# RajeshRk18/exacto

Measured on AMD Instinct MI355X. Metric: ciphertext muls/sec (bfv_mul_and_relin), higher is better.
Workload: dtype u64; 1 GPU; bfv_mul_and_relin, BASELINE configs[2]; ring_degree=4096, ct_limbs=3, limb_bits=60, plain_modulus=65537, gadget_base=65536, gadget_digits=12, batch_per_gpu=1024, global_batch=1024, parallelism=batch-shard x1

## Files before the change

exacto_amd/csrc/ks32.hip:

```cpp
#include "exacto_internal.hpp"
#include "ks32_dev.hpp"

#include <algorithm>

namespace exacto {


template <int LOGN, typename DT, int FORM>
__global__ void __launch_bounds__((1 << LOGN) / 16)
ks32_digit_ntt_kernel(const DT* __restrict__ D16, uint32_t* __restrict__ DS, int G, int S,
                      const Prime32* __restrict__ primes) {
    constexpr int N = 1 << LOGN, T = N / 16;
    __shared__ uint32_t lds[N];
    const int tid = threadIdx.x;
    const uint32_t b = blockIdx.x;
    const int s = (int)(b % (uint32_t)S);
    const long ig = b / (uint32_t)S;
    const Prime32& P = primes[s];
    const DT* src = D16 + ig * N;
    uint32_t x[16];
    constexpr bool SIN = FORM == F32_LAZY && sizeof(DT) == 2;
#pragma unroll
    for (int k = 0; k < 16; ++k) {
        const int d = src[tid + k * T];
        x[k] = SIN ? (uint32_t)d : d < 0 ? P.p + (uint32_t)d : (uint32_t)d;
    }
    fwd32_store<LOGN, FORM, SIN, FORM != F32_LAZY>(x, lds, tid, P, DS + (long)b * N);
}

template <int LOGN, int FORM>
__global__ void __launch_bounds__((1 << LOGN) / 16)
ks32_key_kernel(const u64* __restrict__ K, uint32_t* __restrict__ RS, int L, int S,
                const Prime32* __restrict__ primes, const PrimeConst* __restrict__ qprimes) {
    constexpr int N = 1 << LOGN, T = N / 16;
    __shared__ uint32_t lds[N];
    const int tid = threadIdx.x;
    const uint32_t b = blockIdx.x;
    const int s = (int)(b % (uint32_t)S);
    const uint32_t row = b / (uint32_t)S;
    const int l = (int)(row % (uint32_t)L);
    const Prime32& P = primes[s];
    const u64 q = qprimes[l].q, half = q >> 1;
    const u64* src = K + (long)row * N;
    uint32_t x[16];
#pragma unroll
    for (int k = 0; k < 16; ++k) {
        const u64 r = src[tid + k * T];
        if (r > half) {
            const uint32_t m = (uint32_t)((q - r) % P.p);
            x[k] = m == 0 ? 0 : P.p - m;
        } else {
            x[k] = (uint32_t)(r % P.p);
        }
    }
    fwd32_store<LOGN, FORM>(x, lds, tid, P, RS + (long)b * N);
}

__global__ void __launch_bounds__(256)
ks32_key_norm_kernel(const u64* __restrict__ K, u64* __restrict__ out, int L, int n,
                     const PrimeConst* __restrict__ qprimes) {
    __shared__ u64 part[256];
    const uint32_t row = blockIdx.x;
    const u64 q = qprimes[row % (uint32_t)L].q, half = q >> 1;
    const u64* src = K + (long)row * n;
    u64 acc = 0;
    for (int j = threadIdx.x; j < n; j += 256) {
        const u64 r = src[j];
        acc += (r > half ? q - r : r) >> 20;
    }
    part[threadIdx.x] = acc;
    __syncthreads();
    for (int w = 128; w > 0; w >>= 1) {
        if ((int)threadIdx.x < w) part[threadIdx.x] += part[threadIdx.x + w];
        __syncthreads();
    }
    if (threadIdx.x == 0) out[row] = part[0];
}

__device__ __forceinline__ uint32_t red_s64(long long x, const Prime32& P) {
    const uint32_t p = P.p;
    const uint32_t hu = (uint32_t)((unsigned long long)x >> 32) ^ 0x80000000u;
    const uint32_t a = red32(shoup32(hu, P.c32, P.c32s, p), p);
    const uint32_t b = red32(red32((uint32_t)x, 2 * p), p);
    return red32(red32(a + b, p) + P.k63, p);
}

__device__ __forceinline__ uint32_t red_s64_lz(long long x, const Prime32& P) {
    const uint32_t p = P.p;
    const uint32_t hu = (uint32_t)((unsigned long long)x >> 32) ^ 0x80000000u;
    const uint32_t a = red32(shoup32(hu, P.c32, P.c32s, p), p);
    const uint32_t lo = (uint32_t)x;
    const uint32_t b = lo - (lo >> 30) * p;
    const uint32_t s = a + b + P.k63;
    return min(s, s - 2 * p);
}

__device__ __forceinline__ long long red_s64_lazy(long long x, const Prime32& P) {
    const uint32_t hu = (uint32_t)((unsigned long long)x >> 32) ^ 0x80000000u;
    const uint32_t a = shoup32(hu, P.c32, P.c32s, P.p);
    return (long long)((unsigned long long)a + (uint32_t)x + P.k63);
}

constexpr int KS_LS = 64;
template <int CLB, int NW, int RUN, bool LZ = false>
__global__ void __launch_bounds__(NW * 64)
ks32_mac_kernel(const int* __restrict__ DS, const int* __restrict__ RS, uint32_t* __restrict__ U,
                int G, int CL, int S, int items, int n, const Prime32* __restrict__ primes) {
    extern __shared__ int kl[];
    constexpr int IG = 4 * NW;
    const int lane = threadIdx.x & (KS_LS - 1);
    const int wave = __builtin_amdgcn_readfirstlane(threadIdx.x / KS_LS);
    const int nb = n / KS_LS;
    const int jb = blockIdx.x % nb;
    const int s = (blockIdx.x / nb) % S;
    const int cl0 = (blockIdx.x / (nb * S)) * CLB;
    const int j = jb * KS_LS + lane;
    const Prime32& P = primes[s];
    for (int rr = wave; rr < G * CLB; rr += NW) {
        const int g = rr / CLB, c = rr - g * CLB;
        kl[rr * KS_LS + lane] = RS[(((long)g * CL + cl0 + c) * S + s) * n + jb * KS_LS + lane];
    }
    __syncthreads();
    const int it_end = min(items, (int)(blockIdx.y + 1) * IG);
    for (int it = blockIdx.y * IG + wave; it < it_end; it += NW) {
        const int* dp = DS + ((long)it * G * S + s) * n + j;
        long long acc[CLB];
#pragma unroll
        for (int c = 0; c < CLB; ++c) acc[c] = 0;
        for (int g0 = 0; g0 < G; g0 += RUN) {
            int d[RUN];
#pragma unroll
            for (int e = 0; e < RUN; ++e) d[e] = dp[(long)min(g0 + e, G - 1) * S * n];
#pragma unroll
            for (int e = 0; e < RUN; ++e) d[e] = g0 + e < G ? d[e] : 0;
#pragma unroll
            for (int e = 0; e < RUN; ++e) {
                const int* kg = kl + (min(g0 + e, G - 1) * CLB) * KS_LS + lane;
#pragma unroll
                for (int c = 0; c < CLB; ++c) acc[c] += (long long)d[e] * kg[c * KS_LS];
            }
            if (g0 + RUN < G) {
#pragma unroll
                for (int c = 0; c < CLB; ++c) acc[c] = red_s64_lazy(acc[c], P);
            }
        }
#pragma unroll
        for (int c = 0; c < CLB; ++c)
            U[(((long)it * CL + cl0 + c) * S + s) * n + j] = LZ ? red_s64_lz(acc[c], P) : red_s64(acc[c], P);
    }
}

template <int LOGN, int S, bool LAZY, bool FPC>
__global__ void __launch_bounds__((1 << LOGN) / 16)
ks32_crt_kernel(const uint32_t* __restrict__ U, u64* __restrict__ R, long r_stride, int L,
                const Ks32Tables* __restrict__ KT, const Prime32* __restrict__ primes,
                const PrimeConst* __restrict__ qprimes) {
    constexpr int N = 1 << LOGN, T = N / 16;
    __shared__ uint32_t lds[N];
    const int tid = threadIdx.x;
    const uint32_t b = blockIdx.x;
    u64 x[16];
    ks32_crt_values<LOGN, S, LAZY, FPC>(x, U, R, r_stride, L, b, lds, tid, KT, primes, qprimes);
    const uint32_t CL = 2 * L;
    const long item = b / CL;
    const __amdgpu_buffer_rsrc_t rd = poly_rsrc(R + item * r_stride + (long)(b - (uint32_t)item * CL) * N, N * 8);
#pragma unroll
    for (int k = 0; k < 16; ++k) buf_st64(rd, x[k], tid * 8, k * T * 8);
}

template <typename OT, typename IT>
__global__ void __launch_bounds__(256)
ks32_digit_sum_kernel(const IT* __restrict__ D, int npairs, const int* __restrict__ term_start,
                      const CombineTerm* __restrict__ terms, OT* __restrict__ out, int d, int gu, int n,
                      int nsh) {
    const uint32_t row = blockIdx.x >> nsh;
    const int j = (int)(blockIdx.x & ((1u << nsh) - 1)) * 2048 + 8 * threadIdx.x;
    const uint32_t g = row % (uint32_t)gu;
    const uint32_t ik = row / (uint32_t)gu;
    const int k = (int)(ik % (uint32_t)d);
    const long item = ik / (uint32_t)d;
    int acc[8] = {0, 0, 0, 0, 0, 0, 0, 0};
    for (int t = term_start[k]; t < term_start[k + 1]; ++t) {
        const IT* src = D + ((item * npairs + terms[t].pair) * gu + g) * (long)n + j;
        if constexpr (sizeof(IT) == 2) {
            const uint4 w = *reinterpret_cast<const uint4*>(src);
            const uint32_t v[4] = {w.x, w.y, w.z, w.w};
#pragma unroll
            for (int h = 0; h < 4; ++h) {
                acc[2 * h] += (int)(int16_t)(v[h] & 0xFFFF);
                acc[2 * h + 1] += (int)(int16_t)(v[h] >> 16);
            }
        } else {
            const uint2 w = *reinterpret_cast<const uint2*>(src);
            const uint32_t v[2] = {w.x, w.y};
#pragma unroll
            for (int h = 0; h < 8; ++h) acc[h] += (int)(int8_t)(v[h >> 2] >> (8 * (h & 3)));
        }
    }
    if constexpr (sizeof(OT) == 2) {
        uint4 o;
        uint32_t* op = &o.x;
#pragma unroll
        for (int h = 0; h < 4; ++h) op[h] = ((uint32_t)acc[2 * h] & 0xFFFF) | ((uint32_t)acc[2 * h + 1] << 16);
        *reinterpret_cast<uint4*>(out + (long)row * n + j) = o;
    } else {
        int4* o4 = reinterpret_cast<int4*>(out + (long)row * n + j);
        o4[0] = make_int4(acc[0], acc[1], acc[2], acc[3]);
        o4[1] = make_int4(acc[4], acc[5], acc[6], acc[7]);
    }
}


#define FORM_SWITCH(form, CALL)                          \
    switch (form) {                                      \
        case F32_LAZY: CALL(F32_LAZY); break;            \
        case F32_NARROW: CALL(F32_NARROW); break;        \
        default: CALL(F32_WIDE); break;                  \
    }

template <int LOGN>
static void ks32_launch_digits(const void* D, bool wide, uint32_t* DS, int items, int G, int S, const Prime32* primes,
                               int form, hipStream_t st) {
    const dim3 grid((unsigned)((long)items * G * S)), block((1 << LOGN) / 16);
#define DIG_(F_)                                                                                                \
    do {                                                                                                        \
        if (wide)                                                                                               \
            EXACTO_LAUNCH((ks32_digit_ntt_kernel<LOGN, int32_t, F_>), grid, block, 0, st, (const int32_t*)D, \
                               DS, G, S, primes);                                                               \
        else                                                                                                    \
            EXACTO_LAUNCH((ks32_digit_ntt_kernel<LOGN, int16_t, F_>), grid, block, 0, st, (const int16_t*)D, \
                               DS, G, S, primes);                                                               \
    } while (0)
    FORM_SWITCH(form, DIG_)
#undef DIG_
}

template <int LOGN>
static void ks32_launch_key(const u64* K, uint32_t* RS, long rows, int L, int S, const Prime32* primes,
                            const PrimeConst* qprimes, int form, hipStream_t st) {
#define KEY_(F_) EXACTO_LAUNCH((ks32_key_kernel<LOGN, F_>), dim3((unsigned)(rows * S)), dim3((1 << LOGN) / 16), 0, \
                                    st, K, RS, L, S, primes, qprimes)
    FORM_SWITCH(form, KEY_)
#undef KEY_
}

template <int LOGN, bool LAZY>
static void ks32_launch_crt(const uint32_t* U, u64* R, long r_stride, int items, int L, int S, const Ks32Tables* KT,
                            const Prime32* primes, const PrimeConst* qprimes, hipStream_t st, bool fpc) {
    const dim3 grid((unsigned)((long)items * 2 * L)), block((1 << LOGN) / 16);
#define CRT_(S_, F_) EXACTO_LAUNCH((ks32_crt_kernel<LOGN, S_, LAZY, F_>), grid, block, 0, st, U, R, r_stride, L, KT, \
                                   primes, qprimes)
    if (S == 2) {
        if (fpc) CRT_(2, true); else CRT_(2, false);
    } else if (S == 3) {
        if (fpc) CRT_(3, true); else CRT_(3, false);
    } else {
        if (fpc) CRT_(4, true); else CRT_(4, false);
    }
#undef CRT_
}

#define KS32_SWITCH(logn, CALL)                  \
    switch (logn) {                              \
        case 10: CALL(10); break;                \
        case 11: CALL(11); break;                \
        case 12: CALL(12); break;                \
        case 13: CALL(13); break;                \
        case 14: CALL(14); break;                \
        default: break;                          \
    }

void ks32_digits(const int16_t* D16, uint32_t* DS, int items, int G, int S, int logn, const Prime32* primes, int form,
                 hipStream_t st) {
    if (items <= 0) return;
#define CALL(L_) ks32_launch_digits<L_>(D16, false, DS, items, G, S, primes, form, st)
    KS32_SWITCH(logn, CALL)
#undef CALL
}

void ks32_digits32(const int32_t* D, uint32_t* DS, int items, int G, int S, int logn, const Prime32* primes, int form,
                   hipStream_t st) {
    if (items <= 0) return;
#define CALL(L_) ks32_launch_digits<L_>(D, true, DS, items, G, S, primes, form, st)
    KS32_SWITCH(logn, CALL)
#undef CALL
}

void ks32_key(const u64* K, uint32_t* RS, long rows, int L, int S, int logn, const Prime32* primes,
              const PrimeConst* qprimes, int form, hipStream_t st) {
    if (rows <= 0) return;
#define CALL(L_) ks32_launch_key<L_>(K, RS, rows, L, S, primes, qprimes, form, st)
    KS32_SWITCH(logn, CALL)
#undef CALL
}

void ks32_key_norms(const u64* K, u64* out, long rows, int L, int n, const PrimeConst* qprimes, hipStream_t st) {
    if (rows <= 0) return;
    EXACTO_LAUNCH(ks32_key_norm_kernel, dim3((unsigned)rows), dim3(256), 0, st, K, out, L, n, qprimes);
}

void ks32_mac(const uint32_t* DS, const uint32_t* RS, uint32_t* U, int items, int G, int L, int S, int n,
              const Prime32* primes, int mac_form, hipStream_t st) {
    if (items <= 0) return;
    const int CL = 2 * L;
    int CLB = CL;
    while (CLB > 1 && (CL % CLB != 0 || (size_t)G * CLB * KS_LS * sizeof(int) > 65536)) --CLB;
    const size_t lds = (size_t)G * CLB * KS_LS * sizeof(int);
    const int NW = lds > 32768 ? 8 : 4;
    const dim3 grid((unsigned)((n / KS_LS) * S * (CL / CLB)), (unsigned)((items + 4 * NW - 1) / (4 * NW)));
    const int* ds = reinterpret_cast<const int*>(DS);
    const int* rs = reinterpret_cast<const int*>(RS);
#define MAC_(C_, W_, R_, Z_) EXACTO_LAUNCH((ks32_mac_kernel<C_, W_, R_, Z_>), grid, dim3(W_ * 64), lds, st, ds, rs, U, G, CL, S, items, n, primes)
#define MAC(C_)                                                  \
    do {                                                         \
        if (mac_form == 2) { if (NW == 8) MAC_(C_, 8, 12, true); else MAC_(C_, 4, 12, true); } \
        else if (mac_form == 1) { if (NW == 8) MAC_(C_, 8, 12, false); else MAC_(C_, 4, 12, false); } \
        else { if (NW == 8) MAC_(C_, 8, 7, false); else MAC_(C_, 4, 7, false); }          \
    } while (0)
    switch (CLB) {
        case 8: MAC(8); break;
        case 6: MAC(6); break;
        case 4: MAC(4); break;
        case 3: MAC(3); break;
        case 2: MAC(2); break;
        default: MAC(1); break;
    }
#undef MAC
#undef MAC_
}

void ks32_digit_sum(const void* D, bool in8, int npairs, const int* term_start, const CombineTerm* terms, void* out,
                    bool wide, int items, int d, int gu, int n, hipStream_t st) {
    const long rows = (long)items * d * gu;
    if (rows <= 0) return;
    const int nb = n >= 2048 ? n / 2048 : 1;
    const dim3 grid((unsigned)(rows * nb)), block(n >= 2048 ? 256 : n / 8);
    const int nsh = __builtin_ctz((unsigned)nb);
#define DSUM_(OT, IT) EXACTO_LAUNCH((ks32_digit_sum_kernel<OT, IT>), grid, block, 0, st, (const IT*)D, npairs, \
                                         term_start, terms, (OT*)out, d, gu, n, nsh)
    if (wide) {
        if (in8) DSUM_(int32_t, int8_t); else DSUM_(int32_t, int16_t);
    } else {
        if (in8) DSUM_(int16_t, int8_t); else DSUM_(int16_t, int16_t);
    }
#undef DSUM_
}

void ks32_crt(const uint32_t* U, u64* R, long r_stride, int items, int L, int S, int logn, const Ks32Tables* KT,
              const Prime32* primes, const PrimeConst* qprimes, int form, hipStream_t st, bool fpc) {
    if (items <= 0) return;
    fpc = fpc && (S <= 3 || form != F32_WIDE);
#define CALL(L_)                                                                                                \
    do {                                                                                                        \
        if (form == F32_LAZY) ks32_launch_crt<L_, true>(U, R, r_stride, items, L, S, KT, primes, qprimes, st, fpc); \
        else ks32_launch_crt<L_, false>(U, R, r_stride, items, L, S, KT, primes, qprimes, st, fpc);                \
    } while (0)
    KS32_SWITCH(logn, CALL)
#undef CALL
}

}
```

exacto_amd/csrc/ks32_dev.hpp:

```cpp
#pragma once
#include "exacto_internal.hpp"
#include "bufmem.hpp"

namespace exacto {

typedef const uint2 __attribute__((address_space(1)))* Tw32;
__device__ __forceinline__ Tw32 tw32(const uint2* p) { return (Tw32)p; }

__device__ __forceinline__ uint32_t shoup32(uint32_t x, uint32_t w, uint32_t ws, uint32_t p) {
    return x * w - __umulhi(x, ws) * p;
}

__device__ __forceinline__ uint32_t red32(uint32_t x, uint32_t p) { return min(x, x - p); }

__device__ __forceinline__ int swz32(int j) { return j ^ ((j >> 4) & 15) ^ (((j >> 8) & 1) << 4); }

template <int LO>
__device__ __forceinline__ int eidx(int tid, int k) {
    return ((tid >> LO) << (LO + 4)) | (k << LO) | (tid & ((1 << LO) - 1));
}

__device__ __forceinline__ void lds_sync() { asm volatile("s_waitcnt lgkmcnt(0)\n\ts_barrier" ::: "memory"); }

template <int LO>
__device__ __forceinline__ void lds32_store(uint32_t* lds, const uint32_t (&x)[16], int tid) {
    char* lb = reinterpret_cast<char*>(lds);
    const int b = swz32(eidx<LO>(tid, 0)) << 2;
#pragma unroll
    for (int k = 0; k < 16; ++k) *reinterpret_cast<uint32_t*>(lb + (b ^ (swz32(k << LO) << 2))) = x[k];
}

template <int LO>
__device__ __forceinline__ void lds32_load(const uint32_t* lds, uint32_t (&x)[16], int tid) {
    const char* lb = reinterpret_cast<const char*>(lds);
    const int b = swz32(eidx<LO>(tid, 0)) << 2;
#pragma unroll
    for (int k = 0; k < 16; ++k) x[k] = *reinterpret_cast<const uint32_t*>(lb + (b ^ (swz32(k << LO) << 2)));
}


__device__ __forceinline__ u64 mad64(uint32_t a, uint32_t b, u64 c) {
    u64 r, carry;
    asm("v_mad_u64_u32 %0, %1, %2, %3, %4" : "=v"(r), "=s"(carry) : "v"(a), "v"(b), "v"(c));
    return r;
}

__device__ __forceinline__ u64 lo_only(uint32_t x) {
    typedef uint32_t u32x2 __attribute__((ext_vector_type(2)));
    u32x2 v = __builtin_nondeterministic_value(v);
    v.x = x;
    return __builtin_bit_cast(u64, v);
}

enum { F32_WIDE = 0, F32_NARROW = 1, F32_LAZY = 2 };

template <int LOGN, int LO, int BHI, int FORM, bool CANON = false, bool SIN = false>
__device__ __forceinline__ void fwd32_round(uint32_t (&x)[16], int tid, Tw32 tw, uint32_t p) {
    constexpr int N = 1 << LOGN;
    const int thigh = (LO + 4 >= LOGN) ? 0 : (tid >> LO);
    const uint32_t p2 = 2 * p, np = 0u - p;
    static_assert(!SIN || (FORM == F32_LAZY && CANON && BHI == LOGN - 1), "signed inputs: lazy round 0 only");
    if constexpr (SIN) {
        const uint2 t = make_uint2(tw[1].x, tw[1].y);
        const uint32_t c = red32(shoup32(1u << 15, t.x, t.y, p), p);
        const uint32_t k1 = (p - c) < (1u << 15) ? 2 * p - c : p - c;
        const uint32_t k2 = c < (1u << 15) ? c + 3 * p : c + p2;
        const uint32_t kd = k2 - k1;
#pragma unroll
        for (int m = 0; m < 8; ++m) {
            const uint32_t XK = x[m] + k1, Y = x[m + 8] + (1u << 15);
            const uint32_t qh = __umulhi(Y, t.y);
            const uint32_t o0 = (uint32_t)mad64(qh, np, mad64(Y, t.x, lo_only(XK)));
            uint32_t x2;
            asm("v_lshl_add_u32 %0, %1, 1, %2" : "=v"(x2) : "v"(XK), "v"(kd));
            x[m] = o0;
            x[m + 8] = x2 - o0;
        }
    }
#pragma unroll
    for (int b = SIN ? BHI - 1 : BHI; b >= LO; --b) {
        const int lb = b - LO, half = 1 << lb;
        const int base = (N >> (b + 1)) + (thigh << (LO + 3 - b));
#pragma unroll
        for (int g = 0; g < (8 >> lb); ++g) {
            const uint2 t = make_uint2(tw[base + g].x, tw[base + g].y);
#pragma unroll
            for (int m = 0; m < half; ++m) {
                const int k0 = g * 2 * half + m, k1 = k0 + half;
                if constexpr (FORM != F32_WIDE) {
                    const uint32_t X = (CANON && b == BHI) ? x[k0]
                                       : FORM == F32_LAZY ? min(x[k0], x[k0] - p2)
                                                          : red32(min(x[k0], x[k0] - p2), p);
                    const uint32_t qh = __umulhi(x[k1], t.y);
                    const uint32_t o0 = (uint32_t)mad64(qh, np, mad64(x[k1], t.x, lo_only(X)));
                    x[k0] = o0;
                    x[k1] = 2 * X + p2 - o0;
                } else {
                    const uint32_t X = red32(x[k0], p);
                    const uint32_t T = red32(shoup32(x[k1], t.x, t.y, p), p);
                    x[k0] = X + T;
                    x[k1] = X + p - T;
                }
            }
        }
    }
}

template <int LOGN, int R, int FORM, bool SIN = false>
__device__ __forceinline__ void fwd32_rounds(uint32_t (&x)[16], uint32_t* lds, int tid, Tw32 tw, uint32_t p) {
    constexpr int LO = (LOGN - 4 * (R + 1)) > 0 ? (LOGN - 4 * (R + 1)) : 0;
    constexpr int BHI = LOGN - 1 - 4 * R;
    if constexpr (R > 0) {
        constexpr int PLO = (LOGN - 4 * R) > 0 ? (LOGN - 4 * R) : 0;
        lds_sync();
        lds32_store<PLO>(lds, x, tid);
        lds_sync();
        lds32_load<LO>(lds, x, tid);
    }
    fwd32_round<LOGN, LO, BHI, FORM, R == 0, SIN && R == 0>(x, tid, tw, p);
    if constexpr (LO > 0) fwd32_rounds<LOGN, R + 1, FORM>(x, lds, tid, tw, p);
}

template <int LOGN, int FORM, bool SIN = false, bool BAL = true>
__device__ __forceinline__ void fwd32_store(uint32_t (&x)[16], uint32_t* lds, int tid, const Prime32& P,
                                            uint32_t* __restrict__ dst) {
    constexpr int T = (1 << LOGN) / 16;
    const uint32_t p = P.p, half = p >> 1;
    static_assert(BAL || FORM == F32_LAZY, "canonical digit residues: lazy primes only (MAC bound)");
    fwd32_rounds<LOGN, 0, FORM, SIN>(x, lds, tid, tw32(P.tw_fwd), p);
#pragma unroll
    for (int k = 0; k < 16; ++k)
        x[k] = FORM == F32_WIDE ? red32(x[k], p) : red32(min(x[k], x[k] - 2 * p), p);
    if constexpr (BAL) {
#pragma unroll
        for (int k = 0; k < 16; ++k) x[k] = x[k] > half ? x[k] - p : x[k];
    }
    const __amdgpu_buffer_rsrc_t rd = poly_rsrc(dst, T * 16 * 4);
#pragma unroll
    for (int k = 0; k < 16; ++k) buf_st32(rd, x[k], tid * 4, k * T * 4);
}


template <int LOGN, int LO, int BLO, int BHI, bool LAZY, bool OUT2P = false, bool FOLD = false>
__device__ __forceinline__ void inv32_round(uint32_t (&x)[16], int tid, const Prime32& P) {
    constexpr int N = 1 << LOGN;
    const uint32_t p = P.p, p2 = 2 * p;
    const uint32_t ni = FOLD ? P.fn_inv : P.n_inv, nis = FOLD ? P.fn_inv_s : P.n_inv_s;
    const uint32_t lw = FOLD ? P.flast_w : P.last_w, lws = FOLD ? P.flast_ws : P.last_ws;
    const Tw32 twi = tw32(P.tw_inv);
    const int thigh = (LO + 4 >= LOGN) ? 0 : (tid >> LO);
#pragma unroll
    for (int b = BLO; b <= BHI; ++b) {
        const int lb = b - LO, half = 1 << lb;
        const int base = (N >> (b + 1)) + (thigh << (LO + 3 - b));
#pragma unroll
        for (int g = 0; g < (8 >> lb); ++g) {
            uint2 t = make_uint2(0, 0);
            if (b != LOGN - 1) t = make_uint2(twi[base + g].x, twi[base + g].y);
#pragma unroll
            for (int m = 0; m < half; ++m) {
                const int k0 = g * 2 * half + m, k1 = k0 + half;
                if constexpr (LAZY) {
                    const uint32_t U = x[k0], V = x[k1];
                    if (b == LOGN - 1) {
                        x[k0] = shoup32(U + V, ni, nis, p);
                        x[k1] = shoup32(U + p2 - V, lw, lws, p);
                        if constexpr (!OUT2P) {
                            x[k0] = red32(x[k0], p);
                            x[k1] = red32(x[k1], p);
                        }
                    } else {
                        const uint32_t sum = U + V;
                        x[k0] = min(sum, sum - p2);
                        x[k1] = shoup32(U + p2 - V, t.x, t.y, p);
                    }
                } else {
                    const uint32_t U = red32(x[k0], p), V = red32(x[k1], p);
                    if (b == LOGN - 1) {
                        x[k0] = shoup32(U + V, ni, nis, p);
                        x[k1] = shoup32(U + p - V, lw, lws, p);
                        if constexpr (!OUT2P) {
                            x[k0] = red32(x[k0], p);
                            x[k1] = red32(x[k1], p);
                        }
                    } else {
                        x[k0] = U + V;
                        x[k1] = shoup32(U + p - V, t.x, t.y, p);
                    }
                }
            }
        }
    }
}

template <int LOGN, int R, bool LAZY, bool OUT2P = false, bool FOLD = false>
__device__ __forceinline__ void inv32_rounds(uint32_t (&x)[16], uint32_t* lds, int tid, const Prime32& P) {
    constexpr int LO = (4 * R) < (LOGN - 4) ? 4 * R : LOGN - 4;
    constexpr int BLO = 4 * R;
    constexpr int BHI = (4 * R + 3) < (LOGN - 1) ? 4 * R + 3 : LOGN - 1;
    if constexpr (R > 0) {
        constexpr int PLO = (4 * (R - 1)) < (LOGN - 4) ? 4 * (R - 1) : LOGN - 4;
        lds_sync();
        lds32_store<PLO>(lds, x, tid);
        lds_sync();
        lds32_load<LO>(lds, x, tid);
    }
    inv32_round<LOGN, LO, BLO, BHI, LAZY, OUT2P, FOLD>(x, tid, P);
    if constexpr (BHI < LOGN - 1) inv32_rounds<LOGN, R + 1, LAZY, OUT2P, FOLD>(x, lds, tid, P);
}

template <int S, bool LAZY = false>
__device__ __forceinline__ u64 ks32_lift_one(const uint32_t (&v)[S], u64 r, const uint32_t (&pr)[S],
                                             const uint32_t (&hp)[S], const Ks32Tables* __restrict__ KT, u64 q,
                                             uint32_t dq, u64 negP) {
    uint32_t a[S];
#pragma unroll
    for (int s = 0; s < S; ++s) {
        const uint32_t ps = pr[s];
        uint32_t t = v[s];
#pragma unroll
        for (int kk = 0; kk < s; ++kk) {
            t = LAZY ? t + 2 * ps - a[kk]
                     : t + ps - red32(a[kk], ps);
            t = red32(shoup32(t, KT->ginv[s][kk], KT->ginv_s[s][kk], ps), ps);
        }
        a[s] = t;
    }
    bool gt = false, eq = true;
#pragma unroll
    for (int s = S - 1; s >= 0; --s) {
        gt = gt || (eq && a[s] > hp[s]);
        eq = eq && a[s] == hp[s];
    }
    u64 t = a[S - 1];
#pragma unroll
    for (int s = S - 2; s >= 0; --s) {
        const u64 lo = (u64)(uint32_t)t * pr[s] + a[s];
        const u64 hi = (u64)(uint32_t)(t >> 32) * pr[s] + (lo >> 32);
        const u64 l60 = ((hi & 0x0FFFFFFFull) << 32) | (uint32_t)lo;
        t = l60 + (hi >> 28) * dq;
    }
    if (gt) t += negP;
    return reduce_near60(t + r, q);
}

template <int S>
__device__ __forceinline__ u64 ks32_fpc_one(const uint32_t (&y)[S], u64 r, const double (&ip)[S],
                                            const uint32_t (&c0)[S], const uint32_t (&c1)[S], uint32_t n0,
                                            uint32_t n1, u64 q, uint32_t dq) {
    static_assert(S <= 4, "A0, A1 < 2^64: S <= 3, or S = 4 with p < 2^32 / 3 (ks32_crt)");
    double f = (double)y[0] * ip[0];
#pragma unroll
    for (int s = 1; s < S; ++s) f = __builtin_fma((double)y[s], ip[s], f);
    const uint32_t al = (uint32_t)__builtin_rint(f);
    u64 a0 = (u64)al * n0, a1 = (u64)al * n1;
#pragma unroll
    for (int s = 0; s < S; ++s) {
        a0 += (u64)y[s] * c0[s];
        a1 += (u64)y[s] * c1[s];
    }
    const u64 h = a1 >> 30;
    const u64 l30 = (a1 & ((1ull << 30) - 1)) << 30;
    const u64 t = a0 + l30 + (u64)(uint32_t)h * dq + ((u64)((uint32_t)(h >> 32) * dq) << 32);
    return reduce_near60(t + r, q);
}

template <int LOGN, int S, bool LAZY, bool FPC = false>
__device__ __forceinline__ void ks32_crt_values(u64 (&x)[16], const uint32_t* __restrict__ U, const u64* __restrict__ R,
                                                long r_stride, int L, uint32_t b, uint32_t* lds, int tid,
                                                const Ks32Tables* __restrict__ KT, const Prime32* __restrict__ primes,
                                                const PrimeConst* __restrict__ qprimes) {
    constexpr int N = 1 << LOGN, T = N / 16;
    const uint32_t CL = 2 * L;
    const long item = b / CL;
    const int cl = (int)(b - (uint32_t)item * CL);
    const int l = cl % L;
    uint32_t v[S][16];
#pragma unroll
    for (int s = 0; s < S; ++s) {
        const __amdgpu_buffer_rsrc_t rs = poly_rsrc(U + ((long)b * S + s) * N, N * 4);
#pragma unroll
        for (int k = 0; k < 16; ++k) v[s][k] = buf_ld32(rs, tid * 4, k * T * 4);
        if constexpr (FPC) inv32_rounds<LOGN, 0, LAZY, true, true>(v[s], lds, tid, primes[s]);
        else if (s == 0) inv32_rounds<LOGN, 0, LAZY>(v[s], lds, tid, primes[s]);
        else inv32_rounds<LOGN, 0, LAZY, LAZY>(v[s], lds, tid, primes[s]);
    }
    const u64 q = qprimes[l].q;
    const uint32_t dq = (uint32_t)((1ull << 60) - q);
    const __amdgpu_buffer_rsrc_t rr = poly_rsrc(R + item * r_stride + (long)cl * N, N * 8);
    if constexpr (FPC) {
#pragma unroll
        for (int s = 0; s < S; ++s)
#pragma unroll
            for (int k = 0; k < 16; ++k) asm volatile("" : "+v"(v[s][k]));
        double ip[S];
        uint32_t c0[S], c1[S];
#pragma unroll
        for (int s = 0; s < S; ++s) {
            ip[s] = primes[s].inv_p;
            c0[s] = KT->fpc_c[l][s][0];
            c1[s] = KT->fpc_c[l][s][1];
        }
        const uint32_t n0 = KT->fpc_n[l][0], n1 = KT->fpc_n[l][1];
#pragma unroll
        for (int k = 0; k < 16; ++k) {
            uint32_t vk[S];
#pragma unroll
            for (int s = 0; s < S; ++s) vk[s] = v[s][k];
            x[k] = ks32_fpc_one<S>(vk, buf_ld64(rr, tid * 8, k * T * 8), ip, c0, c1, n0, n1, q, dq);
        }
        return;
    }
    uint32_t pr[S], hp[S];
#pragma unroll
    for (int s = 0; s < S; ++s) {
        pr[s] = primes[s].p;
        hp[s] = KT->halfP[s];
    }
    const u64 negP = KT->negP[l];
#pragma unroll
    for (int k = 0; k < 16; ++k) {
        uint32_t vk[S];
#pragma unroll
        for (int s = 0; s < S; ++s) vk[s] = v[s][k];
        x[k] = ks32_lift_one<S, LAZY>(vk, buf_ld64(rr, tid * 8, k * T * 8), pr, hp, KT, q, dq, negP);
    }
}

}
```

Measured before the change: 488,600 bfv_mul_and_relin/s.

## Park CRT row values in LDS and prefetch next rows during inverse NTT

Adds a PARK variant of the keyswitch CRT kernel for N=4096 that spills most of the first residue row's inverse-NTT output into shared memory instead of holding all S rows in registers. Loads for the next residue row, or the output accumulator, are issued before the final inverse-NTT round, and lifting constants are hoisted out of the per-element loop. The aim is to raise occupancy (launch bound hint of 5) and overlap global loads with compute. In exchange it uses extra LDS per block and adds scheduling barriers that may constrain the compiler.

```diff
diff --git a/exacto_amd/csrc/ks32.hip b/exacto_amd/csrc/ks32.hip
--- a/exacto_amd/csrc/ks32.hip
+++ b/exacto_amd/csrc/ks32.hip
@@ -150,8 +150,8 @@
     }
 }
 
-template <int LOGN, int S, bool LAZY, bool FPC>
-__global__ void __launch_bounds__((1 << LOGN) / 16)
+template <int LOGN, int S, bool LAZY, bool FPC, bool PARK>
+__global__ void __launch_bounds__((1 << LOGN) / 16, PARK ? 5 : 0)
 ks32_crt_kernel(const uint32_t* __restrict__ U, u64* __restrict__ R, long r_stride, int L,
                 const Ks32Tables* __restrict__ KT, const Prime32* __restrict__ primes,
                 const PrimeConst* __restrict__ qprimes) {
@@ -159,13 +159,19 @@
     __shared__ uint32_t lds[N];
     const int tid = threadIdx.x;
     const uint32_t b = blockIdx.x;
-    u64 x[16];
-    ks32_crt_values<LOGN, S, LAZY, FPC>(x, U, R, r_stride, L, b, lds, tid, KT, primes, qprimes);
-    const uint32_t CL = 2 * L;
-    const long item = b / CL;
-    const __amdgpu_buffer_rsrc_t rd = poly_rsrc(R + item * r_stride + (long)(b - (uint32_t)item * CL) * N, N * 8);
-#pragma unroll
-    for (int k = 0; k < 16; ++k) buf_st64(rd, x[k], tid * 8, k * T * 8);
+    if constexpr (PARK) {
+        __shared__ uint32_t park[KS32_PARK * T];
+        ks32_crt_park<LOGN, S, LAZY, FPC>(U, R, r_stride, L, b, lds, park, tid, KT, primes, qprimes);
+    } else {
+        u64 x[16];
+        ks32_crt_values<LOGN, S, LAZY, FPC>(x, U, R, r_stride, L, b, lds, tid, KT, primes, qprimes);
+        const uint32_t CL = 2 * L;
+        const long item = b / CL;
+        const __amdgpu_buffer_rsrc_t rd =
+            poly_rsrc(R + item * r_stride + (long)(b - (uint32_t)item * CL) * N, N * 8);
+#pragma unroll
+        for (int k = 0; k < 16; ++k) buf_st64(rd, x[k], tid * 8, k * T * 8);
+    }
 }
 
 template <typename OT, typename IT>
@@ -248,8 +254,8 @@
 static void ks32_launch_crt(const uint32_t* U, u64* R, long r_stride, int items, int L, int S, const Ks32Tables* KT,
                             const Prime32* primes, const PrimeConst* qprimes, hipStream_t st, bool fpc) {
     const dim3 grid((unsigned)((long)items * 2 * L)), block((1 << LOGN) / 16);
-#define CRT_(S_, F_) EXACTO_LAUNCH((ks32_crt_kernel<LOGN, S_, LAZY, F_>), grid, block, 0, st, U, R, r_stride, L, KT, \
-                                   primes, qprimes)
+#define CRT_(S_, F_) EXACTO_LAUNCH((ks32_crt_kernel<LOGN, S_, LAZY, F_, ks32_crt_parks(LOGN)>), grid, block, 0, st, U, R, \
+                                   r_stride, L, KT, primes, qprimes)
     if (S == 2) {
         if (fpc) CRT_(2, true); else CRT_(2, false);
     } else if (S == 3) {
diff --git a/exacto_amd/csrc/ks32_dev.hpp b/exacto_amd/csrc/ks32_dev.hpp
--- a/exacto_amd/csrc/ks32_dev.hpp
+++ b/exacto_amd/csrc/ks32_dev.hpp
@@ -193,26 +193,32 @@
     }
 }
 
-template <int LOGN, int R, bool LAZY, bool OUT2P = false, bool FOLD = false>
-__device__ __forceinline__ void inv32_rounds(uint32_t (&x)[16], uint32_t* lds, int tid, const Prime32& P) {
+struct NoPre {
+    __device__ __forceinline__ void operator()() const {}
+};
+
+template <int LOGN, int R, bool LAZY, bool OUT2P = false, bool FOLD = false, class PRE = NoPre>
+__device__ __forceinline__ void inv32_rounds(uint32_t (&x)[16], uint32_t* lds, int tid, const Prime32& P,
+                                             PRE pre = PRE()) {
     constexpr int LO = (4 * R) < (LOGN - 4) ? 4 * R : LOGN - 4;
     constexpr int BLO = 4 * R;
     constexpr int BHI = (4 * R + 3) < (LOGN - 1) ? 4 * R + 3 : LOGN - 1;
     if constexpr (R > 0) {
         constexpr int PLO = (4 * (R - 1)) < (LOGN - 4) ? 4 * (R - 1) : LOGN - 4;
+        if constexpr (BHI == LOGN - 1) pre();
         lds_sync();
         lds32_store<PLO>(lds, x, tid);
         lds_sync();
         lds32_load<LO>(lds, x, tid);
     }
     inv32_round<LOGN, LO, BLO, BHI, LAZY, OUT2P, FOLD>(x, tid, P);
-    if constexpr (BHI < LOGN - 1) inv32_rounds<LOGN, R + 1, LAZY, OUT2P, FOLD>(x, lds, tid, P);
+    if constexpr (BHI < LOGN - 1) inv32_rounds<LOGN, R + 1, LAZY, OUT2P, FOLD, PRE>(x, lds, tid, P, pre);
 }
 
 template <int S, bool LAZY = false>
-__device__ __forceinline__ u64 ks32_lift_one(const uint32_t (&v)[S], u64 r, const uint32_t (&pr)[S],
-                                             const uint32_t (&hp)[S], const Ks32Tables* __restrict__ KT, u64 q,
-                                             uint32_t dq, u64 negP) {
+__device__ __forceinline__ u64 ks32_lift_gi(const uint32_t (&v)[S], u64 r, const uint32_t (&pr)[S],
+                                            const uint32_t (&hp)[S], const uint32_t (&gi)[S][S],
+                                            const uint32_t (&gis)[S][S], u64 q, uint32_t dq, u64 negP) {
     uint32_t a[S];
 #pragma unroll
     for (int s = 0; s < S; ++s) {
@@ -222,7 +228,7 @@
         for (int kk = 0; kk < s; ++kk) {
             t = LAZY ? t + 2 * ps - a[kk]
                      : t + ps - red32(a[kk], ps);
-            t = red32(shoup32(t, KT->ginv[s][kk], KT->ginv_s[s][kk], ps), ps);
+            t = red32(shoup32(t, gi[s][kk], gis[s][kk], ps), ps);
         }
         a[s] = t;
     }
@@ -242,6 +248,27 @@
     }
     if (gt) t += negP;
     return reduce_near60(t + r, q);
+}
+
+template <int S>
+__device__ __forceinline__ void ks32_lift_consts(uint32_t (&gi)[S][S], uint32_t (&gis)[S][S],
+                                                 const Ks32Tables* __restrict__ KT) {
+#pragma unroll
+    for (int s = 0; s < S; ++s)
+#pragma unroll
+        for (int kk = 0; kk < S; ++kk) {
+            gi[s][kk] = kk < s ? KT->ginv[s][kk] : 0;
+            gis[s][kk] = kk < s ? KT->ginv_s[s][kk] : 0;
+        }
+}
+
+template <int S, bool LAZY = false>
+__device__ __forceinline__ u64 ks32_lift_one(const uint32_t (&v)[S], u64 r, const uint32_t (&pr)[S],
+                                             const uint32_t (&hp)[S], const Ks32Tables* __restrict__ KT, u64 q,
+                                             uint32_t dq, u64 negP) {
+    uint32_t gi[S][S], gis[S][S];
+    ks32_lift_consts<S>(gi, gis, KT);
+    return ks32_lift_gi<S, LAZY>(v, r, pr, hp, gi, gis, q, dq, negP);
 }
 
 template <int S>
@@ -327,4 +354,121 @@
     }
 }
 
-}
+constexpr int KS32_PARK = 15;
+
+#ifndef EXACTO_CRT_PARK
+#define EXACTO_CRT_PARK 1
+#endif
+
+constexpr bool ks32_crt_parks(int logn) { return EXACTO_CRT_PARK != 0 && logn == 12; }
+
+template <int LOGN, int S, bool LAZY, bool FPC, int SI>
+__device__ __forceinline__ void ks32_park_rows(uint32_t (&v)[S][16], u64 (&r)[16], const uint32_t* __restrict__ U,
+                                               uint32_t b, __amdgpu_buffer_rsrc_t rr, uint32_t* lds, uint32_t* park,
+                                               int tid, const Prime32* __restrict__ primes) {
+    constexpr int N = 1 << LOGN, T = N / 16;
+    auto pre = [&]() {
+        if constexpr (SI + 1 < S) {
+            const __amdgpu_buffer_rsrc_t rs = poly_rsrc(U + ((long)b * S + SI + 1) * N, N * 4);
+#pragma unroll
+            for (int k = 0; k < 16; ++k) v[SI + 1][k] = buf_ld32(rs, tid * 4, k * T * 4);
+        } else {
+#pragma unroll
+            for (int k = 0; k < 8; ++k) r[k] = buf_ld64(rr, tid * 8, k * T * 8);
+        }
+    };
+    int t = tid;
+    if constexpr (SI >= 2) asm volatile("" : "+v"(t));
+    if constexpr (FPC) inv32_rounds<LOGN, 0, LAZY, true, true>(v[SI], lds, t, primes[SI], pre);
+    else if constexpr (SI == 0) inv32_rounds<LOGN, 0, LAZY, false, false>(v[SI], lds, t, primes[SI], pre);
+    else inv32_rounds<LOGN, 0, LAZY, LAZY, false>(v[SI], lds, t, primes[SI], pre);
+    if constexpr (SI == 0) {
+#pragma unroll
+        for (int k = 0; k < KS32_PARK; ++k) park[k * T + tid] = v[0][k];
+    }
+    if constexpr (SI + 1 < S) ks32_park_rows<LOGN, S, LAZY, FPC, SI + 1>(v, r, U, b, rr, lds, park, tid, primes);
+}
+
+template <int LOGN, int S, bool LAZY, bool FPC>
+__device__ __forceinline__ void ks32_crt_park(const uint32_t* __restrict__ U, u64* __restrict__ R, long r_stride,
+                                              int L, uint32_t b, uint32_t* lds, uint32_t* park, int tid,
+                                              const Ks32Tables* __restrict__ KT, const Prime32* __restrict__ primes,
+                                              const PrimeConst* __restrict__ qprimes) {
+    constexpr int N = 1 << LOGN, T = N / 16;
+    static_assert(S >= 2, "the parked words are read back after a later row's barriers");
+    const uint32_t CL = 2 * L;
+    const long item = b / CL;
+    const int cl = (int)(b - (uint32_t)item * CL);
+    const int l = cl % L;
+    const __amdgpu_buffer_rsrc_t rr = poly_rsrc(R + item * r_stride + (long)cl * N, N * 8);
+    const u64 q = qprimes[l].q;
+    const uint32_t dq = (uint32_t)((1ull << 60) - q);
+    double ip[S];
+    uint32_t c0[S], c1[S], pr[S], hp[S], gi[S][S], gis[S][S];
+    uint32_t n0 = 0, n1 = 0;
+    u64 negP = 0;
+    if constexpr (FPC) {
+#pragma unroll
+        for (int s = 0; s < S; ++s) {
+            ip[s] = primes[s].inv_p;
+            c0[s] = KT->fpc_c[l][s][0];
+            c1[s] = KT->fpc_c[l][s][1];
+        }
+        n0 = KT->fpc_n[l][0];
+        n1 = KT->fpc_n[l][1];
+    } else {
+#pragma unroll
+        for (int s = 0; s < S; ++s) {
+            pr[s] = primes[s].p;
+            hp[s] = KT->halfP[s];
+        }
+        negP = KT->negP[l];
+        ks32_lift_consts<S>(gi, gis, KT);
+    }
+    uint32_t v[S][16];
+    u64 r[16];
+    {
+        const __amdgpu_buffer_rsrc_t rs = poly_rsrc(U + (long)b * S * N, N * 4);
+#pragma unroll
+        for (int k = 0; k < 16; ++k) v[0][k] = buf_ld32(rs, tid * 4, k * T * 4);
+    }
+    ks32_park_rows<LOGN, S, LAZY, FPC, 0>(v, r, U, b, rr, lds, park, tid, primes);
+    if constexpr (FPC) {
+#pragma unroll
+        for (int s = 0; s < S; ++s)
+#pragma unroll
+            for (int k = s == 0 ? KS32_PARK : 0; k < 16; ++k) asm volatile("" : "+v"(v[s][k]));
+    }
+    constexpr int GRP = (!FPC && S == 4) ? 1 : 2;
+    auto parked = [&](int k) { return k < KS32_PARK ? park[k * T + tid] : v[0][k]; };
+    uint32_t pk[GRP];
+#pragma unroll
+    for (int e = 0; e < GRP; ++e) pk[e] = parked(e);
+#pragma unroll
+    for (int g = 0; g < 16 / GRP; ++g) {
+        __builtin_amdgcn_sched_barrier(0);
+        uint32_t pn[GRP];
+#pragma unroll
+        for (int e = 0; e < GRP; ++e) pn[e] = g + 1 < 16 / GRP ? parked(GRP * (g + 1) + e) : 0;
+        if (g == 2 / GRP) {
+#pragma unroll
+            for (int k = 8; k < 16; ++k) r[k] = buf_ld64(rr, tid * 8, k * T * 8);
+        }
+#pragma unroll
+        for (int e = 0; e < GRP; ++e) {
+            const int k = GRP * g + e;
+            uint32_t vk[S];
+            vk[0] = pk[e];
+#pragma unroll
+            for (int s = 1; s < S; ++s) vk[s] = v[s][k];
+            u64 x;
+            if constexpr (FPC) x = ks32_fpc_one<S>(vk, r[k], ip, c0, c1, n0, n1, q, dq);
+            else x = ks32_lift_gi<S, LAZY>(vk, r[k], pr, hp, gi, gis, q, dq, negP);
+            buf_st64(rr, x, tid * 8, k * T * 8);
+        }
+#pragma unroll
+        for (int e = 0; e < GRP; ++e) pk[e] = pn[e];
+    }
+}
+
+}
```

New measurement: 491,700 bfv_mul_and_relin/s, median of 6. About the same (+0.6%).
